# Blaizzy/mlx-audio-swift

Measured on AMD Instinct MI355X. Metric: audio-seconds/sec (TTS gen+codec decode), Orpheus-3B batch 32 per GPU: value = whole-job aggregate over n_gpus, value_per_gpu = value / n_gpus, higher is better.
Workload: dtype bf16

## Files before the change

### include/mi_speech_debug.h

```cpp
#ifndef MI_SPEECH_DEBUG_H
#define MI_SPEECH_DEBUG_H
#include "mi_speech.h"
#ifdef __cplusplus
extern "C" {
#endif

mis_status mis_debug_launch_floor(int device, int n_kernels, int mode, int reps, double* us_per_kernel);
int32_t mis_debug_choose_split(int32_t items, int32_t k_tiles, int32_t waves_per_item, int32_t s_max);
mis_status mis_debug_occupy_cus(int device, int blocks, int threads, double seconds);
mis_status mis_debug_occupy_wait(void);
int32_t mis_debug_device_cus(int device);
int32_t mis_debug_sampler_failures(void);
int64_t mis_debug_whisper_weight_bytes(const mis_whisper* c);
mis_status mis_debug_mimi_decoder_tap(mis_mimi* m, const int32_t* codes, int batch, int n_q, int T, int stage, float* out, int64_t capacity,
                                      int32_t* channels, int64_t* length);

mis_status mis_debug_gemm_skinny(int device, const uint16_t* W, const uint16_t* W2, const uint16_t* X, const uint16_t* bias, int M, int N, int K,
                                 int epi, int R, int ksb, int U, int S, float* out, int64_t capacity, int32_t* report);
mis_status mis_debug_gemm_skinny_q(int device, int bits, int sb_dtype, const uint32_t* wq, const uint16_t* scales, const uint16_t* biases,
                                   const uint32_t* wq2, const uint16_t* scales2, const uint16_t* biases2, const uint16_t* X, const uint16_t* bias,
                                   int M, int N, int K, int epi, int R, int ksb, int S, float* out, int64_t capacity, int32_t* report);
mis_status mis_debug_gemm_pf(int device, const uint16_t* W, const uint16_t* W2, const uint16_t* X, const uint16_t* h, int M, int N, int K, int epi,
                             float* out, int64_t capacity, int32_t* report);

typedef struct mis_debug_attn_args {
    int32_t batch, Mpad, S, Nqkv, H, Hkv, D, Smax;
    int32_t cache_rows, append_only, first_schedule, cross, cross_len, out_ld, rope_in_dtype;
    int32_t qp_S, qp_KT;
    float scale, qk_eps, qp_eps;
    const float* qkv_part;
    const int32_t* pos;
    const uint8_t* active;
    const float *rope_cos, *rope_sin;
    const uint16_t *qnorm_w, *knorm_w;
    const uint16_t* qp_w;
    const uint16_t* qp_bias;
    const float* qp_slabs;
    const uint16_t *qp_h_in, *qp_lnw, *qp_lnb;
    const uint16_t *kcache, *vtcache;
    uint16_t *kcache_out, *vtcache_out;
    float* out;
    uint16_t* qp_h_out;
    int32_t* report;
} mis_debug_attn_args;
mis_status mis_debug_attn_decode(int device, const mis_debug_attn_args* args);

mis_status mis_debug_token_engine(mis_tts* lm, const int32_t* prompt, int n_prompt, int n_new, int xcds, const mis_gen_params* sampling,
                                  int stop_id, int32_t* next_tokens, float* logits_out, float* hidden_out, int32_t* counts, double* ms_out);

mis_status mis_debug_marvis_forced_logits(mis_marvis* c, const int32_t* tokens, const uint8_t* mask, const int32_t* prompt_lens, int P,
                                          int batch, const mis_marvis_params* params, const int32_t* forced, int F, float* logits_out,
                                          int32_t* sampled_out, int32_t* n_frames);
mis_status mis_debug_marvis_sample_logits(int device, const float* logits, int batch, int vocab, float temperature, float top_p,
                                          uint64_t seed, int64_t row_offset, int frame, int slot, int K, int32_t* tokens_out);
mis_status mis_debug_marvis_rope_tables(int head_dim, float theta, float factor, float low_freq_factor, float high_freq_factor,
                                        float old_context_len, int n_pos, float* cos_out, float* sin_out);

mis_status mis_debug_moonshine_stem_tap(mis_moonshine* c, const float* pcm, const int64_t* lens, int batch, int64_t stride, int stage,
                                        float* out, int64_t capacity, int64_t* dims);

mis_status mis_debug_smartturn_tap(mis_smartturn* c, int stage, float* out, int64_t capacity);
mis_status mis_debug_smartturn_timing(const mis_smartturn* c, float* ms);

mis_status mis_debug_ecapa_lid_timing(const mis_ecapa_lid* c, float* ms);

#ifdef __cplusplus
}
#endif
#endif
```

### mlx-audio-swift_amd/_lib.py

```python
from __future__ import annotations

import ctypes as C
import os

_HERE = os.path.dirname(os.path.abspath(__file__))
LIB_PATH = os.environ.get("MIS_LIB_PATH") or os.path.join(_HERE, "libmi_speech.so")

MIS_OK = 0
STATUS_NAMES = {0: "ok", 1: "modelNotInitialized", 2: "generationFailed", 3: "invalidInput",
                4: "audioDecodingFailed", 5: "audioEncodingFailed", 6: "cancelled", 7: "device"}
MIS_F32, MIS_F16, MIS_BF16, MIS_I32 = 0, 1, 2, 3
EVENT_TOKEN, EVENT_INFO, EVENT_AUDIO = 0, 1, 2


class SnacConfigC(C.Structure):
    _fields_ = [("sampling_rate", C.c_int32), ("latent_dim", C.c_int32), ("decoder_dim", C.c_int32),
                ("n_decoder_rates", C.c_int32), ("decoder_rates", C.c_int32 * 8), ("codebook_size", C.c_int32),
                ("codebook_dim", C.c_int32), ("n_codebooks", C.c_int32), ("vq_strides", C.c_int32 * 8),
                ("noise", C.c_int32), ("depthwise", C.c_int32), ("attn_window_size", C.c_int32)]


class LmConfigC(C.Structure):
    _fields_ = [("hidden_size", C.c_int32), ("num_hidden_layers", C.c_int32), ("intermediate_size", C.c_int32),
                ("num_attention_heads", C.c_int32), ("num_key_value_heads", C.c_int32), ("head_dim", C.c_int32),
# ... 321 lines not shown
    "mis_encodec_hop_length": (C.c_int, [_P]),
    "mis_encodec_decode_frame": (C.c_int, [_P, _P, C.c_int, C.c_int, C.c_int, _P, _P]),
    "mis_encodec_debug_tap": (C.c_int, [_P, _P, C.c_int, C.c_int, C.c_int, C.c_int, _P, C.c_int64, C.POINTER(C.c_int32),
                                        C.POINTER(C.c_int64)]),
    "mis_mimi_202407": (None, [C.c_int, C.POINTER(MimiConfigC)]),
    "mis_mimi_create": (C.c_int, [C.POINTER(MimiConfigC), C.c_int, C.POINTER(_P)]),
    "mis_mimi_set_tensor": (C.c_int, [_P, C.c_char_p, _P, C.c_int, C.POINTER(C.c_int64), C.c_int]),
    "mis_mimi_finalize": (C.c_int, [_P]),
    "mis_mimi_destroy": (None, [_P]),
    "mis_mimi_num_samples": (C.c_int64, [_P, C.c_int]),
    "mis_mimi_decode": (C.c_int, [_P, _P, C.c_int, C.c_int, C.c_int, _P]),
    "mis_mimi_encode_num_frames": (C.c_int64, [_P, C.c_int64]),
    "mis_mimi_encode": (C.c_int, [_P, _P, C.c_int, C.c_int64, C.c_int, _P]),
    "mis_mimi_decode_stream_begin": (C.c_int, [_P, C.c_int]),
    "mis_mimi_decode_stream_step": (C.c_int, [_P, _P, C.c_int, C.c_int, _P]),
    "mis_mimi_decode_stream_end": (C.c_int, [_P]),
    "mis_marvis_create": (C.c_int, [C.POINTER(MarvisConfigC), C.c_int, C.POINTER(_P)]),
    "mis_marvis_set_tensor": (C.c_int, [_P, C.c_char_p, _P, C.c_int, C.POINTER(C.c_int64), C.c_int]),
    "mis_marvis_set_tensor_quantized": (C.c_int, [_P, C.c_char_p, _P, _P, _P, C.c_int, C.c_int64, C.c_int64, C.c_int, C.c_int]),
    "mis_marvis_init_synthetic": (C.c_int, [_P, C.c_uint64]),
    "mis_marvis_init_synthetic_quantized": (C.c_int, [_P, C.c_uint64, C.c_int]),
    "mis_marvis_finalize": (C.c_int, [_P]),
    "mis_marvis_destroy": (None, [_P]),
    "mis_marvis_backbone": (_P, [_P]),
    "mis_marvis_decoder": (_P, [_P]),
    "mis_marvis_launches_per_frame": (C.c_int, [_P]),
    "mis_marvis_generate_codes": (C.c_int, [_P, _P, _P, _P, C.c_int, C.c_int, C.POINTER(MarvisParamsC), _P, C.POINTER(_P),
                                            C.POINTER(C.c_int64), _P]),
    "mis_marvis_generate": (C.c_int, [_P, _P, _P, _P, _P, C.c_int, C.c_int, C.POINTER(MarvisParamsC), _P, C.POINTER(_P),
                                      C.POINTER(C.c_int64), _P, C.POINTER(_P), C.POINTER(C.c_int64), _P, C.c_int, _P, _P, _P]),
}

class AttnDebugArgsC(C.Structure):
    _fields_ = ([(n, C.c_int32) for n in ("batch", "Mpad", "S", "Nqkv", "H", "Hkv", "D", "Smax", "cache_rows", "append_only", "first_schedule",
                                          "cross", "cross_len", "out_ld", "rope_in_dtype", "qp_S", "qp_KT")] +
                [(n, C.c_float) for n in ("scale", "qk_eps", "qp_eps")] +
                [(n, _P) for n in ("qkv_part", "pos", "active", "rope_cos", "rope_sin", "qnorm_w", "knorm_w", "qp_w", "qp_bias", "qp_slabs",
                                   "qp_h_in", "qp_lnw", "qp_lnb", "kcache", "vtcache", "kcache_out", "vtcache_out", "out", "qp_h_out", "report")])


DEBUG_SYMBOLS = {
    "mis_debug_launch_floor": (C.c_int, [C.c_int, C.c_int, C.c_int, C.c_int, C.POINTER(C.c_double)]),
    "mis_debug_occupy_cus": (C.c_int, [C.c_int, C.c_int, C.c_int, C.c_double]),
    "mis_debug_occupy_wait": (C.c_int, []),
    "mis_debug_device_cus": (C.c_int32, [C.c_int]),
    "mis_debug_sampler_failures": (C.c_int32, []),
    "mis_debug_choose_split": (C.c_int32, [C.c_int32, C.c_int32, C.c_int32, C.c_int32]),
    "mis_debug_gemm_skinny": (C.c_int, [C.c_int, _P, _P, _P, _P, C.c_int, C.c_int, C.c_int, C.c_int, C.c_int, C.c_int, C.c_int, C.c_int, _P,
                                        C.c_int64, _P]),
    "mis_debug_gemm_skinny_q": (C.c_int, [C.c_int, C.c_int, C.c_int, _P, _P, _P, _P, _P, _P, _P, _P, C.c_int, C.c_int, C.c_int, C.c_int, C.c_int,
                                          C.c_int, C.c_int, _P, C.c_int64, _P]),
    "mis_debug_gemm_pf": (C.c_int, [C.c_int, _P, _P, _P, _P, C.c_int, C.c_int, C.c_int, C.c_int, _P, C.c_int64, _P]),
    "mis_debug_attn_decode": (C.c_int, [C.c_int, C.POINTER(AttnDebugArgsC)]),
    "mis_debug_token_engine": (C.c_int, [_P, _P, C.c_int, C.c_int, C.c_int, _P, C.c_int, _P, _P, _P, _P, C.POINTER(C.c_double)]),
    "mis_debug_whisper_weight_bytes": (C.c_int64, [_P]),
    "mis_debug_mimi_decoder_tap": (C.c_int, [_P, _P, C.c_int, C.c_int, C.c_int, C.c_int, _P, C.c_int64, C.POINTER(C.c_int32),
                                             C.POINTER(C.c_int64)]),
    "mis_debug_marvis_forced_logits": (C.c_int, [_P, _P, _P, _P, C.c_int, C.c_int, C.POINTER(MarvisParamsC), _P, C.c_int, _P, _P, _P]),
    "mis_debug_marvis_sample_logits": (C.c_int, [C.c_int, _P, C.c_int, C.c_int, C.c_float, C.c_float, C.c_uint64, C.c_int64, C.c_int,
                                                 C.c_int, C.c_int, _P]),
    "mis_debug_moonshine_stem_tap": (C.c_int, [_P, _P, _P, C.c_int, C.c_int64, C.c_int, _P, C.c_int64, _P]),
    "mis_debug_smartturn_tap": (C.c_int, [_P, C.c_int, _P, C.c_int64]),
    "mis_debug_smartturn_timing": (C.c_int, [_P, _P]),
    "mis_debug_ecapa_lid_timing": (C.c_int, [_P, _P]),
    "mis_debug_marvis_rope_tables": (C.c_int, [C.c_int, C.c_float, C.c_float, C.c_float, C.c_float, C.c_float, C.c_int, _P, _P]),
}

_lib = None


class MisLibraryMissing(RuntimeError):
    pass


def lib():
    global _lib
    if _lib is None:
        if not os.path.exists(LIB_PATH):
            raise MisLibraryMissing(
                f"{LIB_PATH} not found: build it with `python -c 'import __graft_entry__ as g; g.build()'` "
                "(hipcc --offload-arch=gfx950). There is no CPU fallback.")
        try:
            import torch
        except Exception:
            pass
        l = C.CDLL(LIB_PATH)
        for name, (res, args) in list(SYMBOLS.items()) + list(DEBUG_SYMBOLS.items()):
            fn = getattr(l, name)
            fn.restype = res
            fn.argtypes = args
        _lib = l
    return _lib


def last_error() -> str:
    m = lib().mis_last_error()
    return m.decode("utf-8", "replace") if m else ""
```

### mlx-audio-swift_amd/csrc/lm_kernels.hip

```cpp
#include <hip/hip_fp16.h>
#include "common.h"
#include <algorithm>
#include <type_traits>
#include <string>
#include "lm_kernels.h"



__global__ void k_convert_to_bf16(const void* __restrict__ src, int dtype, bf16_t* __restrict__ dst, size_t n) {
    size_t i = (size_t)blockIdx.x * blockDim.x + threadIdx.x;
    if (i >= n) return;
    if (dtype == MIS_F32) dst[i] = f32_to_bf16(((const float*)src)[i]);
    else if (dtype == MIS_F16) dst[i] = f32_to_bf16((float)((const _Float16*)src)[i]);
    else dst[i] = ((const bf16_t*)src)[i];
}

__global__ void k_bf16_to_f32(const bf16_t* __restrict__ src, float* __restrict__ dst, size_t n) {
    size_t i = (size_t)blockIdx.x * blockDim.x + threadIdx.x;
    if (i < n) dst[i] = bf16_to_f32(src[i]);
}

__global__ void k_pack_weight(const bf16_t* __restrict__ src, bf16_t* __restrict__ dst, int N, int K, int NT,
                              int tile_stride, int tile_offset) {
    int KT = K / 32;
// ... 225 lines not shown
        for (int k = 0; k < RR_MAXC; ++k) {
            int i = c0 + tid + k * RR_THREADS;
            keep[k] = 0.0f;
            if (i < N) {
                float o = bf16_round_f32(acc[k]);
                float hn = bf16_round_f32(hv[k] + o);
                h[(size_t)m * N + i] = f32_to_bf16(hn);
                keep[k] = hn;
                ss += hn * hn;
            }
        }
    }
    if (ln_bias) {
        float sum = 0.0f;
        if (N <= RR_THREADS * RR_MAXC) {
#pragma unroll
            for (int k = 0; k < RR_MAXC; ++k) sum += keep[k];
        } else {
            for (int i = tid; i < N; i += RR_THREADS) sum += bf16_to_f32(h[(size_t)m * N + i]);
        }
        const float mean = block_sum_1024(sum, red) / (float)N;
        float sq = 0.0f;
        if (N <= RR_THREADS * RR_MAXC) {
#pragma unroll
            for (int k = 0; k < RR_MAXC; ++k) {
                int i = tid + k * RR_THREADS;
                if (i < N) { float dlt = keep[k] - mean; sq += dlt * dlt; }
            }
        } else {
            for (int i = tid; i < N; i += RR_THREADS) { float dlt = bf16_to_f32(h[(size_t)m * N + i]) - mean; sq += dlt * dlt; }
        }
        const float rstd = 1.0f / sqrtf(block_sum_1024(sq, red) / (float)N + eps);
        for (int i = tid; i < N; i += RR_THREADS) {
            float f = bf16_to_f32(h[(size_t)m * N + i]);
            x[xpk_index(m, i, MT)] = f32_to_bf16((f - mean) * rstd * bf16_to_f32(wnorm[i]) + bf16_to_f32(ln_bias[i]));
        }
        return;
    }
    float tot = block_sum_1024(ss, red);
    float inv = 1.0f / sqrtf(tot / (float)N + eps);
    if (N <= RR_THREADS * RR_MAXC) {
#pragma unroll
        for (int k = 0; k < RR_MAXC; ++k) {
            int i = tid + k * RR_THREADS;
            if (i < N) x[xpk_index(m, i, MT)] = f32_to_bf16(wv[k] * bf16_round_f32(keep[k] * inv));
        }
    } else {
        for (int i = tid; i < N; i += RR_THREADS) {
            float f = bf16_to_f32(h[(size_t)m * N + i]);
            x[xpk_index(m, i, MT)] = f32_to_bf16(bf16_to_f32(wnorm[i]) * bf16_round_f32(f * inv));
        }
    }
}
template <int SG, bool LN>
__global__ void __launch_bounds__(1024) k_glue4(const float* __restrict__ slabs, int S, int Mpad, int N, bf16_t* __restrict__ h,
                                                const bf16_t* __restrict__ wnorm, bf16_t* __restrict__ x, float eps,
                                                const bf16_t* __restrict__ ln_bias) {
    __shared__ float red[16];
    const int m = blockIdx.x, tid = threadIdx.x, nth = blockDim.x;
    const int MT = Mpad >> 4;
    const int c4 = tid < (N >> 2) ? tid : (N >> 2) - 1;
    const bool live = tid < (N >> 2);
    unsigned long long hq, wq, bq = 0;
    f32x4_t v[SG];
    {
        const bf16_t* hp = h + (size_t)m * N + 4 * c4;
        const bf16_t* wp = wnorm + 4 * c4;
        asm volatile("global_load_dwordx2 %0, %1, off" : "=v"(hq) : "v"(hp));
        asm volatile("global_load_dwordx2 %0, %1, off" : "=v"(wq) : "v"(wp));
        if constexpr (LN) {
            const bf16_t* bp = ln_bias + 4 * c4;
            asm volatile("global_load_dwordx2 %0, %1, off" : "=v"(bq) : "v"(bp));
        }
#pragma unroll
        for (int j = 0; j < SG; ++j) {
            const int sj = j < S ? j : S - 1;
            const float* sp = slabs + ((size_t)sj * Mpad + m) * N + 4 * c4;
            asm volatile("global_load_dwordx4 %0, %1, off" : "=v"(v[j]) : "v"(sp));
        }
        if constexpr (SG == 2) asm volatile("s_waitcnt vmcnt(0)" : "+v"(hq), "+v"(wq), "+v"(v[0]), "+v"(v[1]));
        else if constexpr (SG == 4) asm volatile("s_waitcnt vmcnt(0)" : "+v"(hq), "+v"(wq), "+v"(v[0]), "+v"(v[1]), "+v"(v[2]), "+v"(v[3]));
        else asm volatile("s_waitcnt vmcnt(0)" : "+v"(hq), "+v"(wq), "+v"(v[0]), "+v"(v[1]), "+v"(v[2]), "+v"(v[3]), "+v"(v[4]), "+v"(v[5]),
                          "+v"(v[6]), "+v"(v[7]));
        if constexpr (LN) asm volatile("" : "+v"(bq));
    }
    float acc[4] = {0.f, 0.f, 0.f, 0.f};
#pragma unroll
    for (int j = 0; j < SG; ++j) {
        const bool on = j < S;
        acc[0] += on ? v[j][0] : 0.0f; acc[1] += on ? v[j][1] : 0.0f; acc[2] += on ? v[j][2] : 0.0f; acc[3] += on ? v[j][3] : 0.0f;
    }
    const uint32_t hq0 = (uint32_t)hq, hq1 = (uint32_t)(hq >> 32);
    const float hv[4] = {bf16_to_f32((bf16_t)(hq0 & 0xffffu)), bf16_to_f32((bf16_t)(hq0 >> 16)), bf16_to_f32((bf16_t)(hq1 & 0xffffu)),
                         bf16_to_f32((bf16_t)(hq1 >> 16))};
    const uint32_t wq0 = (uint32_t)wq, wq1 = (uint32_t)(wq >> 32);
    const float wv[4] = {bf16_to_f32((bf16_t)(wq0 & 0xffffu)), bf16_to_f32((bf16_t)(wq0 >> 16)), bf16_to_f32((bf16_t)(wq1 & 0xffffu)),
                         bf16_to_f32((bf16_t)(wq1 >> 16))};
    float hn[4], ss = 0.0f;
    bf16_t hb[4];
#pragma unroll
    for (int e = 0; e < 4; ++e) {
        hn[e] = bf16_round_f32(hv[e] + bf16_round_f32(acc[e]));
        hb[e] = f32_to_bf16(hn[e]);
        ss += live ? hn[e] * hn[e] : 0.0f;
    }
    if (live) *reinterpret_cast<uint2*>(h + (size_t)m * N + 4 * c4) =
        make_uint2((uint32_t)hb[0] | ((uint32_t)hb[1] << 16), (uint32_t)hb[2] | ((uint32_t)hb[3] << 16));
    if constexpr (LN) {
        float sm = 0.0f;
#pragma unroll
        for (int e = 0; e < 4; ++e) sm += live ? hn[e] : 0.0f;
        sm = wave_sum_dpp(sm);
        if ((tid & 63) == 0) red[tid >> 6] = sm;
        __syncthreads();
        float tot = 0.0f;
        const int nw = nth >> 6;
#pragma unroll
        for (int i = 0; i < 16; ++i) tot += i < nw ? red[i] : 0.0f;
        const float mean = tot / (float)N;
        float sq = 0.0f;
#pragma unroll
        for (int e = 0; e < 4; ++e) { const float dl = hn[e] - mean; sq += live ? dl * dl : 0.0f; }
        sq = wave_sum_dpp(sq);
        __syncthreads();
        if ((tid & 63) == 0) red[tid >> 6] = sq;
        __syncthreads();
        float tq = 0.0f;
#pragma unroll
        for (int i = 0; i < 16; ++i) tq += i < nw ? red[i] : 0.0f;
        const float rstd = 1.0f / sqrtf(tq / (float)N + eps);
        if (live) {
            const uint32_t bq0 = (uint32_t)bq, bq1 = (uint32_t)(bq >> 32);
            const float bv[4] = {bf16_to_f32((bf16_t)(bq0 & 0xffffu)), bf16_to_f32((bf16_t)(bq0 >> 16)), bf16_to_f32((bf16_t)(bq1 & 0xffffu)),
                                 bf16_to_f32((bf16_t)(bq1 >> 16))};
            bf16_t xb[4];
#pragma unroll
            for (int e = 0; e < 4; ++e) xb[e] = f32_to_bf16((hn[e] - mean) * rstd * wv[e] + bv[e]);
            *reinterpret_cast<uint2*>(x + xpk_index(m, 4 * c4, MT)) =
                make_uint2((uint32_t)xb[0] | ((uint32_t)xb[1] << 16), (uint32_t)xb[2] | ((uint32_t)xb[3] << 16));
        }
        return;
    }
    ss = wave_sum_dpp(ss);
    if ((tid & 63) == 0) red[tid >> 6] = ss;
    __syncthreads();
    float tot = 0.0f;
    const int nw = nth >> 6;
#pragma unroll
    for (int i = 0; i < 16; ++i) tot += i < nw ? red[i] : 0.0f;
    const float inv = 1.0f / sqrtf(tot / (float)N + eps);
    if (live) {
        bf16_t xb[4];
#pragma unroll
        for (int e = 0; e < 4; ++e) xb[e] = f32_to_bf16(wv[e] * bf16_round_f32(hn[e] * inv));
        *reinterpret_cast<uint2*>(x + xpk_index(m, 4 * c4, MT)) =
            make_uint2((uint32_t)xb[0] | ((uint32_t)xb[1] << 16), (uint32_t)xb[2] | ((uint32_t)xb[3] << 16));
    }
}

template <int SG, int CPT, bool LN>
__global__ void __launch_bounds__(256) k_glue_cpt(const float* __restrict__ slabs, int S, int Mpad, int N, bf16_t* __restrict__ h,
                                                  const bf16_t* __restrict__ wnorm, bf16_t* __restrict__ x, float eps, const bf16_t* __restrict__ ln_bias) {
    __shared__ float red[4];
    const int m = blockIdx.x, tid = threadIdx.x, nth = blockDim.x;
    const int MT = Mpad >> 4;
    const int nw = nth >> 6;
    unsigned long long hq[CPT], wq[CPT], bq[CPT];
    f32x4_t v[CPT][SG];
#pragma unroll
    for (int g = 0; g < CPT; ++g) {
        const int c4 = tid + g * nth;
        const bf16_t* hp = h + (size_t)m * N + 4 * c4;
        const bf16_t* wp = wnorm + 4 * c4;
        asm volatile("global_load_dwordx2 %0, %1, off" : "=v"(hq[g]) : "v"(hp));
        asm volatile("global_load_dwordx2 %0, %1, off" : "=v"(wq[g]) : "v"(wp));
        if constexpr (LN) {
            const bf16_t* bp = ln_bias + 4 * c4;
            asm volatile("global_load_dwordx2 %0, %1, off" : "=v"(bq[g]) : "v"(bp));
        } else bq[g] = 0;
    }
#pragma unroll
    for (int j = 0; j < SG; ++j) {
        const int sj = j < S ? j : S - 1;
#pragma unroll
        for (int g = 0; g < CPT; ++g) {
            const float* sp = slabs + ((size_t)sj * Mpad + m) * N + 4 * (tid + g * nth);
            asm volatile("global_load_dwordx4 %0, %1, off" : "=v"(v[g][j]) : "v"(sp));
        }
    }
    asm volatile("s_waitcnt vmcnt(0)" ::: "memory");
#pragma unroll
    for (int g = 0; g < CPT; ++g) {
        asm volatile("" : "+v"(hq[g]), "+v"(wq[g]));
        if constexpr (LN) asm volatile("" : "+v"(bq[g]));
#pragma unroll
        for (int j = 0; j < SG; ++j) asm volatile("" : "+v"(v[g][j]));
    }
    auto row_sum = [&](float part, bool again) {
        part = wave_sum_dpp(part);
        if (nw == 1) return part;
        if (again) __syncthreads();
        if ((tid & 63) == 0) red[tid >> 6] = part;
        __syncthreads();
        float tot = 0.0f;
#pragma unroll
        for (int i = 0; i < 4; ++i) tot += i < nw ? red[i] : 0.0f;
        return tot;
    };
    float hn[CPT][4], wv[CPT][4], ss = 0.0f, sm = 0.0f;
#pragma unroll
    for (int g = 0; g < CPT; ++g) {
        float acc[4] = {0.f, 0.f, 0.f, 0.f};
#pragma unroll
        for (int j = 0; j < SG; ++j) {
            const bool on = j < S;
            acc[0] += on ? v[g][j][0] : 0.0f; acc[1] += on ? v[g][j][1] : 0.0f; acc[2] += on ? v[g][j][2] : 0.0f; acc[3] += on ? v[g][j][3] : 0.0f;
        }
        const uint32_t h0 = (uint32_t)hq[g], h1 = (uint32_t)(hq[g] >> 32), w0 = (uint32_t)wq[g], w1 = (uint32_t)(wq[g] >> 32);
        const float hv[4] = {bf16_to_f32((bf16_t)(h0 & 0xffffu)), bf16_to_f32((bf16_t)(h0 >> 16)), bf16_to_f32((bf16_t)(h1 & 0xffffu)), bf16_to_f32((bf16_t)(h1 >> 16))};
        wv[g][0] = bf16_to_f32((bf16_t)(w0 & 0xffffu)); wv[g][1] = bf16_to_f32((bf16_t)(w0 >> 16));
        wv[g][2] = bf16_to_f32((bf16_t)(w1 & 0xffffu)); wv[g][3] = bf16_to_f32((bf16_t)(w1 >> 16));
        bf16_t hb[4];
#pragma unroll
        for (int e = 0; e < 4; ++e) {
            hn[g][e] = bf16_round_f32(hv[e] + bf16_round_f32(acc[e]));
            hb[e] = f32_to_bf16(hn[g][e]);
            ss += hn[g][e] * hn[g][e];
            sm += hn[g][e];
        }
        *reinterpret_cast<uint2*>(h + (size_t)m * N + 4 * (tid + g * nth)) =
            make_uint2((uint32_t)hb[0] | ((uint32_t)hb[1] << 16), (uint32_t)hb[2] | ((uint32_t)hb[3] << 16));
    }
    if constexpr (LN) {
        const float mean = row_sum(sm, false) / (float)N;
        float sq = 0.0f;
#pragma unroll
        for (int g = 0; g < CPT; ++g)
#pragma unroll
            for (int e = 0; e < 4; ++e) { const float dl = hn[g][e] - mean; sq += dl * dl; }
        const float rstd = 1.0f / sqrtf(row_sum(sq, true) / (float)N + eps);
#pragma unroll
// ... 942 lines not shown
        if (xs_nj == 6) xs_run(std::integral_constant<int, 6>{});
        else xs_run(std::integral_constant<int, 5>{});
#undef XS_BIND
    } else {
        for (int tile = wave; tile < n_tiles; tile += 2 * ATT_WAVES) {
            const int tile2 = tile + ATT_WAVES;
            const bool has2 = tile2 < n_tiles;
            if (tile != wave) {
                load_tile(tile, kA, vA);
                if (has2) load_tile(tile2, kB, vB);
            }
            if (tile == new_tile) patch_new_key(kA, vA);
            process(tile, kA, vA);
            if (has2) {
                if (tile2 == new_tile) patch_new_key(kB, vB);
                process(tile2, kB, vB);
            }
        }
    }
    ATT_STAMP(5);
    l_run += __shfl_xor(l_run, 16, 64);
    l_run += __shfl_xor(l_run, 32, 64);
    if (g4 == 0) { sm[wave * 16 + h] = m_run; sl[wave * 16 + h] = l_run; }
#pragma unroll
    for (int r = 0; r < 4; ++r) {
        int head = g4 * 4 + r;
        if (head < G) {
#pragma unroll
            for (int dt = 0; dt < D / 16; ++dt) sO[((size_t)wave * G + head) * D + dt * 16 + h] = O[dt][r];
        }
    }
    __syncthreads();
    ATT_STAMP(6);
    for (int idx = tid; idx < G * D; idx += 512) {
        int head = idx / D, d = idx - head * D;
        float M = -INFINITY;
#pragma unroll
        for (int w = 0; w < ATT_WAVES; ++w) M = fmaxf(M, sm[w * 16 + head]);
        float num = 0.0f, den = 0.0f;
#pragma unroll
        for (int w = 0; w < ATT_WAVES; ++w) {
            float f = __expf(sm[w * 16 + head] - M);
            num += f * sO[((size_t)w * G + head) * D + d];
            den += f * sl[w * 16 + head];
        }
        const bf16_t ov = f32_to_bf16(num / den);
        if (p.out_ld) p.out[(size_t)b * p.out_ld + (kvh * G + head) * D + d] = ov;
        else p.out[xpk_index(b, (kvh * G + head) * D + d, p.Mpad >> 4)] = ov;
    }
    ATT_STAMP(7);
}

#define ATT2_MAX_J 4
__device__ __forceinline__ void att2_issue_tile(const bf16_t* kt, const bf16_t* vt, unsigned voff, bf16x8_t (&ka)[2][4], bf16x8_t (&vb)[8]) {
    const bf16_t* kt1 = kt + 4 * 512;
    const bf16_t* vt1 = vt + 4 * 512;
#define ATT2_NT " nt"
#define ATT2_LD(DST, BASE, OFF) asm volatile("global_load_dwordx4 %0, %1, %2 offset:" #OFF ATT2_NT : "=v"(DST) : "v"(voff), "s"(BASE))
    asm volatile("s_nop 4\n\tglobal_load_dwordx4 %0, %1, %2" ATT2_NT : "=v"(ka[0][0]) : "v"(voff), "s"(kt));
    ATT2_LD(ka[0][1], kt, 1024); ATT2_LD(ka[0][2], kt, 2048); ATT2_LD(ka[0][3], kt, 3072);
    asm volatile("s_nop 4\n\tglobal_load_dwordx4 %0, %1, %2" ATT2_NT : "=v"(ka[1][0]) : "v"(voff), "s"(kt1));
    ATT2_LD(ka[1][1], kt1, 1024); ATT2_LD(ka[1][2], kt1, 2048); ATT2_LD(ka[1][3], kt1, 3072);
    asm volatile("s_nop 4\n\tglobal_load_dwordx4 %0, %1, %2" ATT2_NT : "=v"(vb[0]) : "v"(voff), "s"(vt));
    ATT2_LD(vb[1], vt, 1024); ATT2_LD(vb[2], vt, 2048); ATT2_LD(vb[3], vt, 3072);
    asm volatile("s_nop 4\n\tglobal_load_dwordx4 %0, %1, %2" ATT2_NT : "=v"(vb[4]) : "v"(voff), "s"(vt1));
    ATT2_LD(vb[5], vt1, 1024); ATT2_LD(vb[6], vt1, 2048); ATT2_LD(vb[7], vt1, 3072);
#undef ATT2_LD
}
#define ATT2_VMCNT(CNT) asm volatile("s_waitcnt vmcnt(" #CNT ")" ::: "memory")
#define ATT2_BIND_TILE(KA, VB)                                                                                               \
    asm volatile("" : "+v"(KA[0][0]), "+v"(KA[0][1]), "+v"(KA[0][2]), "+v"(KA[0][3]), "+v"(KA[1][0]), "+v"(KA[1][1]), "+v"(KA[1][2]),  \
                      "+v"(KA[1][3]), "+v"(VB[0]), "+v"(VB[1]), "+v"(VB[2]), "+v"(VB[3]), "+v"(VB[4]), "+v"(VB[5]), "+v"(VB[6]), "+v"(VB[7]))

template <int NS>
__global__ void __launch_bounds__(512) k_attn_decode2(AttnParams p) {
    constexpr int D = 128;
    extern __shared__ __attribute__((aligned(16))) unsigned char smem[];
    const int kvh = blockIdx.x, b = blockIdx.y;
    const int tid = threadIdx.x, lane = tid & 63, wave = __builtin_amdgcn_readfirstlane(tid >> 6);
    const int G = p.H / p.Hkv;
    float* strip = reinterpret_cast<float*>(smem) + (size_t)wave * 7 * D;
    float* sm = reinterpret_cast<float*>(smem) + (size_t)ATT_WAVES * 7 * D;
    float* sl = sm + ATT_WAVES * 16;
    float* sO = sl + ATT_WAVES * 16;

    const uint32_t active_word = reinterpret_cast<const uint32_t*>(p.active)[b >> 2];
    const unsigned char row_active = (unsigned char)((active_word >> (8 * (b & 3))) & 0xffu);
    const int pos = p.pos[b];
    if (!row_active) return;
    const int kv_len = pos + 1;
    const int n_tiles = (kv_len + 31) >> 5;
    const int new_tile = pos >> 5;
    const bool owner = (new_tile & (ATT_WAVES - 1)) == wave;
    const int nj = wave < n_tiles ? (n_tiles - wave + ATT_WAVES - 1) / ATT_WAVES : 0;

    bf16_t* kc = p.kcache + ((size_t)(b * p.Hkv + kvh) * p.Smax) * D;
    bf16_t* vt = p.vtcache + ((size_t)(b * p.Hkv + kvh) * D) * p.Smax;
    const unsigned voff = (unsigned)lane * 16u;
    auto ktile = [&](int tile) { return kc + (size_t)tile * 32 * D; };
    auto vtile = [&](int tile) { return vt + (size_t)tile * 32 * D; };
    const int h = lane & 15, g4 = lane >> 4;
    const int pr = pos & 31;
    const int prow = ((pr >> 3) << 2) | (pr & 3), phalf = (pr >> 2) & 1;
    bf16_t* kro = reinterpret_cast<bf16_t*>(strip + 6 * D);

    f32x4_t O[D / 16];
// ... 86 lines not shown
        __builtin_amdgcn_wave_barrier();
        __builtin_amdgcn_fence(__ATOMIC_ACQUIRE, "wavefront");

#pragma unroll
        for (int dt = 0; dt < D / 16; ++dt) O[dt] = (f32x4_t){0.f, 0.f, 0.f, 0.f};
        m_run = -INFINITY; l_run = 0.0f;
        auto process = [&](int tile, const bf16x8_t (&ka)[2][4], const bf16x8_t (&vb)[8]) {
            const int base = tile * 32;
            f32x4_t S0 = (f32x4_t){0.f, 0.f, 0.f, 0.f}, S1 = S0;
#pragma unroll
            for (int c = 0; c < D / 32; ++c) {
                S0 = __builtin_amdgcn_mfma_f32_16x16x32_bf16(ka[0][c], qf[c], S0, 0, 0, 0);
                S1 = __builtin_amdgcn_mfma_f32_16x16x32_bf16(ka[1][c], qf[c], S1, 0, 0, 0);
            }
            float sc[8];
            float mx = -INFINITY;
#pragma unroll
            for (int e = 0; e < 8; ++e) {
                float v = (e < 4 ? S0[e] : S1[e - 4]) * p.scale;
                v = (base + g4 * 8 + e < kv_len) ? v : -INFINITY;
                sc[e] = v;
                mx = fmaxf(mx, v);
            }
            mx = fmaxf(mx, __shfl_xor(mx, 16, 64));
            mx = fmaxf(mx, __shfl_xor(mx, 32, 64));
            float m_new = fmaxf(m_run, mx);
            float alpha = __expf(m_run - m_new);
            float psum = 0.0f;
            bf16x8_t ph, pl;
#pragma unroll
            for (int e = 0; e < 8; ++e) {
                float pe = __expf(sc[e] - m_new);
                psum += pe;
                bf16_t hi = f32_to_bf16(pe);
                bf16_t lo = f32_to_bf16(pe - bf16_to_f32(hi));
                ph[e] = (short)hi;
                pl[e] = (short)lo;
            }
            l_run = l_run * alpha + psum;
            m_run = m_new;
            float ar[4];
#pragma unroll
            for (int r = 0; r < 4; ++r) ar[r] = __shfl(alpha, g4 * 4 + r, 64);
#pragma unroll
            for (int dt = 0; dt < D / 16; ++dt) {
                f32x4_t o = O[dt];
#pragma unroll
                for (int r = 0; r < 4; ++r) o[r] *= ar[r];
                o = __builtin_amdgcn_mfma_f32_16x16x32_bf16(ph, vb[dt], o, 0, 0, 0);
                o = __builtin_amdgcn_mfma_f32_16x16x32_bf16(pl, vb[dt], o, 0, 0, 0);
                O[dt] = o;
            }
        };
        auto last = [&](int tile, bf16x8_t (&ka)[2][4], bf16x8_t (&vb)[8]) {
            if (owner) {
                if ((lane & 15) == prow) {
                    bf16x8_t* dst = reinterpret_cast<bf16x8_t*>(kc) + ((size_t)new_tile * 2 + phalf) * (D / 32) * 64 + lane;
#pragma unroll
                    for (int c = 0; c < 4; ++c) {
                        const bf16x8_t kn = *reinterpret_cast<const bf16x8_t*>(kro + c * 32 + g4 * 8);
                        if (phalf) ka[1][c] = kn; else ka[0][c] = kn;
                        dst[c * 64] = kn;
                    }
                }
                if ((lane >> 4) == (pr >> 3)) {
#pragma unroll
                    for (int dt = 0; dt < 8; ++dt) {
                        const bf16_t vn = f32_to_bf16(strip[(G + 1) * D + dt * 16 + (lane & 15)]);
#pragma unroll
                        for (int e = 0; e < 8; ++e)
                            if (e == (pr & 7)) vb[dt][e] = (short)vn;
                        vt[(((size_t)new_tile * (D / 16) + dt) * 64 + lane) * 8 + (pr & 7)] = vn;
                    }
                }
            }
            process(tile, ka, vb);
        };
        __builtin_amdgcn_sched_barrier(0);
        if constexpr (NJ >= 2) att2_issue_tile(ktile(wave + ATT_WAVES), vtile(wave + ATT_WAVES), voff, kB, vB);
        if constexpr (NJ >= 1) {
            if constexpr (NJ >= 2) ATT2_VMCNT(16); else ATT2_VMCNT(0);
            ATT2_BIND_TILE(kA, vA);
            __builtin_amdgcn_sched_barrier(0);
            if constexpr (NJ == 1) last(wave, kA, vA); else process(wave, kA, vA);
            __builtin_amdgcn_sched_barrier(0);
        }
        if constexpr (NJ >= 2) {
            if constexpr (NJ >= 3) att2_issue_tile(ktile(wave + 2 * ATT_WAVES), vtile(wave + 2 * ATT_WAVES), voff, kA, vA);
            if constexpr (NJ >= 3) ATT2_VMCNT(16); else ATT2_VMCNT(0);
            ATT2_BIND_TILE(kB, vB);
            __builtin_amdgcn_sched_barrier(0);
            if constexpr (NJ == 2) last(wave + ATT_WAVES, kB, vB); else process(wave + ATT_WAVES, kB, vB);
            __builtin_amdgcn_sched_barrier(0);
        }
        if constexpr (NJ >= 3) {
            if constexpr (NJ >= 4) att2_issue_tile(ktile(wave + 3 * ATT_WAVES), vtile(wave + 3 * ATT_WAVES), voff, kB, vB);
            if constexpr (NJ >= 4) ATT2_VMCNT(16); else ATT2_VMCNT(0);
            ATT2_BIND_TILE(kA, vA);
            __builtin_amdgcn_sched_barrier(0);
            if constexpr (NJ == 3) last(wave + 2 * ATT_WAVES, kA, vA); else process(wave + 2 * ATT_WAVES, kA, vA);
            __builtin_amdgcn_sched_barrier(0);
        }
        if constexpr (NJ >= 4) {
            ATT2_VMCNT(0);
            ATT2_BIND_TILE(kB, vB);
            __builtin_amdgcn_sched_barrier(0);
            last(wave + 3 * ATT_WAVES, kB, vB);
        }
    };
    switch (nj) {
        case 1: run(std::integral_constant<int, 1>{}); break;
        case 2: run(std::integral_constant<int, 2>{}); break;
        case 3: run(std::integral_constant<int, 3>{}); break;
        case 4: run(std::integral_constant<int, 4>{}); break;
        default: run(std::integral_constant<int, 0>{}); break;
    }
    l_run += __shfl_xor(l_run, 16, 64);
    l_run += __shfl_xor(l_run, 32, 64);
    if (g4 == 0) { sm[wave * 16 + h] = m_run; sl[wave * 16 + h] = l_run; }
#pragma unroll
    for (int r = 0; r < 4; ++r) {
        int head = g4 * 4 + r;
        if (head < G) {
#pragma unroll
            for (int dt = 0; dt < D / 16; ++dt) sO[((size_t)wave * G + head) * D + dt * 16 + h] = O[dt][r];
        }
    }
    __syncthreads();
    for (int idx = tid; idx < G * D; idx += 512) {
        int head = idx / D, d = idx - head * D;
        float M = -INFINITY;
#pragma unroll
        for (int w = 0; w < ATT_WAVES; ++w) M = fmaxf(M, sm[w * 16 + head]);
        float num = 0.0f, den = 0.0f;
#pragma unroll
        for (int w = 0; w < ATT_WAVES; ++w) {
            float f = __expf(sm[w * 16 + head] - M);
            num += f * sO[((size_t)w * G + head) * D + d];
            den += f * sl[w * 16 + head];
        }
        const bf16_t ov = f32_to_bf16(num / den);
        if (p.out_ld) p.out[(size_t)b * p.out_ld + (kvh * G + head) * D + d] = ov;
        else p.out[xpk_index(b, (kvh * G + head) * D + d, p.Mpad >> 4)] = ov;
    }
}
static size_t attn2_smem_bytes(int G) { return ((size_t)ATT_WAVES * 7 * 128 + 2 * ATT_WAVES * 16 + (size_t)ATT_WAVES * G * 128) * 4; }

#ifdef MIS_ATTN_TIMING
#include <string.h>
static unsigned long long* g_attn_dbg = nullptr;
static int g_attn_slot = 0;
extern "C" int mis_debug_attn_timing_init() {
    if (!g_attn_dbg) {
        if (hipHostMalloc((void**)&g_attn_dbg, 4096 * 16 * sizeof(unsigned long long), 0) != hipSuccess) return 1;
        memset(g_attn_dbg, 0, 4096 * 16 * 8);
    }
    g_attn_slot = 0;
    return 0;
}
extern "C" int mis_debug_attn_timing(unsigned long long* out, int max_slots) {
    int n = g_attn_slot < max_slots ? g_attn_slot : max_slots;
    if (g_attn_dbg) memcpy(out, g_attn_dbg, (size_t)n * 16 * 8);
    return n;
}
#endif
static int attn_nit(int G, int D) {
    const int n_el = (G + 2) * D;
    return n_el <= 1024 ? 2 : (D == 128 ? 5 : 3);
}
size_t attn_smem_bytes(int G, int D) {
    return (size_t)attn_nit(G, D) * 512 * 4 + 16 * D * 2 + D * 2 + 2 * ATT_WAVES * 16 * 4 + (size_t)ATT_WAVES * G * D * 4;
}

thread_local AttnLaunchInfo g_attn_last_launch;

bool attn_qp_ok(const AttnParams& p) {
    const char* xe = getenv("MIS_ATTN_XS");
    return !(xe && atoi(xe) == 0) && p.cross && p.D == 64 && p.H == p.Hkv && !p.append_only && !p.cache_rows && !p.rope_cos && !p.qnorm_w &&
           (p.cross_len + 31) / 32 >= ATT_WAVES * ATT_XS_MIN_J && (p.cross_len + 31) / 32 <= ATT_WAVES * ATT_XS_MAX_J && p.qp_KT >= 1 &&
           (p.qp_KT + ATT_WAVES - 1) / ATT_WAVES <= ATT_QP_KW && p.qp_KT * 32 == p.H * p.D && p.qp_S >= 1 && p.qp_S <= 8;
}
void launch_attn_decode(const AttnParams& p, int batch, hipStream_t s) {
    int G = p.H / p.Hkv;
    MIS_REQUIRE(G >= 1 && G <= 16 && p.H % p.Hkv == 0, MIS_ERR_INVALID_INPUT, "GQA group size must be 1..16");
    size_t smem = attn_smem_bytes(G, p.D);
    MIS_REQUIRE(smem <= 64 * 1024, MIS_ERR_INVALID_INPUT, "attention LDS footprint too large");
    MIS_REQUIRE(p.qp_w || (p.S >= 1 && p.S <= 8), MIS_ERR_GENERATION_FAILED, "attention prologue reduces at most 8 split-K slabs (got %d)", p.S);
    MIS_REQUIRE(((uintptr_t)p.active & 3) == 0, MIS_ERR_GENERATION_FAILED, "attention: the active-flag array must be 4-byte aligned");
    MIS_REQUIRE(!p.qp_w || attn_qp_ok(p), MIS_ERR_GENERATION_FAILED, "attention: the query-projection prologue does not apply to this launch");
    MIS_REQUIRE(p.Smax >= 32 && p.Smax % 32 == 0, MIS_ERR_INVALID_INPUT, "attention: %d cache positions are not a multiple of the 32-key tile", p.Smax);
    dim3 grid(p.Hkv, batch), block(512);
    const int n_el = (G + 2) * p.D;
    if (!p.first_schedule && !p.cache_rows && !p.append_only && p.D == 128 && !p.cross && p.rope_cos && !p.rope_in_dtype && !p.qnorm_w && p.S <= 4 && G <= 4 && p.Smax <= 32 * ATT_WAVES * ATT2_MAX_J &&
        p.Smax % 32 == 0 && ((uintptr_t)p.qkv_part & 15) == 0 && p.Nqkv % 4 == 0) {
        const size_t sm2 = attn2_smem_bytes(G);
        MIS_REQUIRE((p.Smax / 32 + ATT_WAVES - 1) / ATT_WAVES <= ATT2_MAX_J, MIS_ERR_GENERATION_FAILED,
// ... 43 lines not shown
```

Baseline: 184.1.

## Vectorize attention combine, precompute new KV tile data, use SGPR-base glue loads

The glue residual-RMSNorm kernels now issue loads with a scalar base and a 32-bit vector offset instead of full 64-bit per-lane addresses, which cuts VGPR address arithmetic. The decode attention kernel gathers the new token's K/V values early (prep) and merges them into the last tile with branch-free masked selects, so that work overlaps the outstanding tile loads. The cross-wave combine is also vectorized: each thread handles 8 output columns with 16-byte LDS reads and stores, and the sm/sl layout is transposed to head-major to allow this. A debug entry point for the glue kernel is added. The risks are extra register pressure and the more complex masking logic.

```diff
diff --git a/include/mi_speech_debug.h b/include/mi_speech_debug.h
--- a/include/mi_speech_debug.h
+++ b/include/mi_speech_debug.h
@@ -45,6 +45,9 @@
 } mis_debug_attn_args;
 mis_status mis_debug_attn_decode(int device, const mis_debug_attn_args* args);
 
+mis_status mis_debug_glue(int device, const float* slabs, int S, int Mpad, int N, const uint16_t* h_in, const uint16_t* wnorm,
+                          const uint16_t* ln_bias, float eps, uint16_t* h_out, uint16_t* x_out);
+
 mis_status mis_debug_token_engine(mis_tts* lm, const int32_t* prompt, int n_prompt, int n_new, int xcds, const mis_gen_params* sampling,
                                   int stop_id, int32_t* next_tokens, float* logits_out, float* hidden_out, int32_t* counts, double* ms_out);
 
diff --git a/mlx-audio-swift_amd/_lib.py b/mlx-audio-swift_amd/_lib.py
--- a/mlx-audio-swift_amd/_lib.py
+++ b/mlx-audio-swift_amd/_lib.py
@@ -397,6 +397,7 @@
                                           C.c_int, C.c_int, _P, C.c_int64, _P]),
     "mis_debug_gemm_pf": (C.c_int, [C.c_int, _P, _P, _P, _P, C.c_int, C.c_int, C.c_int, C.c_int, _P, C.c_int64, _P]),
     "mis_debug_attn_decode": (C.c_int, [C.c_int, C.POINTER(AttnDebugArgsC)]),
+    "mis_debug_glue": (C.c_int, [C.c_int, _P, C.c_int, C.c_int, C.c_int, _P, _P, _P, C.c_float, _P, _P]),
     "mis_debug_token_engine": (C.c_int, [_P, _P, C.c_int, C.c_int, C.c_int, _P, C.c_int, _P, _P, _P, _P, C.POINTER(C.c_double)]),
     "mis_debug_whisper_weight_bytes": (C.c_int64, [_P]),
     "mis_debug_mimi_decoder_tap": (C.c_int, [_P, _P, C.c_int, C.c_int, C.c_int, C.c_int, _P, C.c_int64, C.POINTER(C.c_int32),
diff --git a/mlx-audio-swift_amd/csrc/glue_debug.hip b/mlx-audio-swift_amd/csrc/glue_debug.hip
--- /dev/null
+++ b/mlx-audio-swift_amd/csrc/glue_debug.hip
@@ -0,0 +1,34 @@
+#include "common.h"
+#include "lm_kernels.h"
+#include "debug_guard.h"
+#include "../../include/mi_speech_debug.h"
+
+extern "C" mis_status mis_debug_glue(int device, const float* slabs, int S, int Mpad, int N, const uint16_t* h_in, const uint16_t* wnorm,
+                                     const uint16_t* ln_bias, float eps, uint16_t* h_out, uint16_t* x_out) {
+    MIS_API_BEGIN
+    MIS_REQUIRE(slabs && h_in && wnorm && h_out && x_out, MIS_ERR_INVALID_INPUT, "glue: slabs, h, the norm weight and both outputs are required");
+    MIS_REQUIRE(S >= 1 && S <= 64 && Mpad >= 16 && Mpad % 16 == 0 && Mpad <= 64 && N >= 32 && N % 32 == 0 && N <= 16384, MIS_ERR_INVALID_INPUT,
+                "glue: 1 <= S <= 64 slabs, Mpad 16 .. 64 (a multiple of 16), N a multiple of 32 up to 16384");
+    HIP_CHECK(hipSetDevice(device));
+    DevBuf<uint32_t> d_slabs;
+    DevBuf<uint16_t> d_w, d_b;
+    alloc32(d_slabs, slabs, (size_t)S * Mpad * N, F32_NAN);
+    alloc16(d_w, wnorm, N, BF16_NAN);
+    if (ln_bias) alloc16(d_b, ln_bias, N, BF16_NAN);
+    GuardedOut h, x;
+    const size_t bytes = (size_t)Mpad * N * 2;
+    h.alloc(bytes, (size_t)N * 2);
+    x.alloc(bytes, (size_t)N * 2);
+    HIP_CHECK(hipMemcpy(h.p(), h_in, bytes, hipMemcpyHostToDevice));
+    launch_reduce_residual_rmsnorm(reinterpret_cast<const float*>(d_slabs.p), S, Mpad, N, reinterpret_cast<bf16_t*>(h.p()), d_w.p,
+                                   reinterpret_cast<bf16_t*>(x.p()), eps, 0, ln_bias ? d_b.p : nullptr);
+    HIP_CHECK(hipGetLastError());
+    HIP_CHECK(hipDeviceSynchronize());
+    h.check_guards(); x.check_guards();
+    HIP_CHECK(hipMemcpy(h_out, h.p(), bytes, hipMemcpyDeviceToHost));
+    std::vector<uint16_t> pk((size_t)Mpad * N);
+    HIP_CHECK(hipMemcpy(pk.data(), x.p(), bytes, hipMemcpyDeviceToHost));
+    for (int m = 0; m < Mpad; ++m)
+        for (int k = 0; k < N; ++k) x_out[(size_t)m * N + k] = pk[xpk_index(m, k, Mpad >> 4)];
+    MIS_API_END
+}
diff --git a/mlx-audio-swift_amd/csrc/lm_kernels.hip b/mlx-audio-swift_amd/csrc/lm_kernels.hip
--- a/mlx-audio-swift_amd/csrc/lm_kernels.hip
+++ b/mlx-audio-swift_amd/csrc/lm_kernels.hip
@@ -301,6 +301,8 @@
         }
     }
 }
+#define GLUE_LD(OP, DST, VOFF, BASE) asm volatile(OP " %0, %1, %2" : "=v"(DST) : "v"(VOFF), "s"(BASE))
+#define GLUE_LD_S(OP, DST, VOFF, BASE) asm volatile("s_nop 4\n\t" OP " %0, %1, %2" : "=v"(DST) : "v"(VOFF), "s"(BASE))
 template <int SG, bool LN>
 __global__ void __launch_bounds__(1024) k_glue4(const float* __restrict__ slabs, int S, int Mpad, int N, bf16_t* __restrict__ h,
                                                 const bf16_t* __restrict__ wnorm, bf16_t* __restrict__ x, float eps,
@@ -313,19 +315,17 @@
     unsigned long long hq, wq, bq = 0;
     f32x4_t v[SG];
     {
-        const bf16_t* hp = h + (size_t)m * N + 4 * c4;
-        const bf16_t* wp = wnorm + 4 * c4;
-        asm volatile("global_load_dwordx2 %0, %1, off" : "=v"(hq) : "v"(hp));
-        asm volatile("global_load_dwordx2 %0, %1, off" : "=v"(wq) : "v"(wp));
-        if constexpr (LN) {
-            const bf16_t* bp = ln_bias + 4 * c4;
-            asm volatile("global_load_dwordx2 %0, %1, off" : "=v"(bq) : "v"(bp));
-        }
+        const unsigned o8 = 8u * (unsigned)c4, o16 = 16u * (unsigned)c4;
+        const bf16_t* hrow = h + (size_t)m * N;
+        const float* srow = slabs + (size_t)m * N;
+        const size_t slab_stride = (size_t)Mpad * N;
+        GLUE_LD_S("global_load_dwordx2", hq, o8, hrow);
+        GLUE_LD("global_load_dwordx2", wq, o8, wnorm);
+        if constexpr (LN) GLUE_LD("global_load_dwordx2", bq, o8, ln_bias);
 #pragma unroll
         for (int j = 0; j < SG; ++j) {
-            const int sj = j < S ? j : S - 1;
-            const float* sp = slabs + ((size_t)sj * Mpad + m) * N + 4 * c4;
-            asm volatile("global_load_dwordx4 %0, %1, off" : "=v"(v[j]) : "v"(sp));
+            const float* sp = srow + (size_t)(j < S ? j : S - 1) * slab_stride;
+            GLUE_LD("global_load_dwordx4", v[j], o16, sp);
         }
         if constexpr (SG == 2) asm volatile("s_waitcnt vmcnt(0)" : "+v"(hq), "+v"(wq), "+v"(v[0]), "+v"(v[1]));
         else if constexpr (SG == 4) asm volatile("s_waitcnt vmcnt(0)" : "+v"(hq), "+v"(wq), "+v"(v[0]), "+v"(v[1]), "+v"(v[2]), "+v"(v[3]));
@@ -416,26 +416,25 @@
     const int nw = nth >> 6;
     unsigned long long hq[CPT], wq[CPT], bq[CPT];
     f32x4_t v[CPT][SG];
+    unsigned o8[CPT], o16[CPT];
+#pragma unroll
+    for (int g = 0; g < CPT; ++g) { o8[g] = 8u * (unsigned)(tid + g * nth); o16[g] = 2u * o8[g]; }
+    const bf16_t* hrow = h + (size_t)m * N;
+    const float* srow = slabs + (size_t)m * N;
+    const size_t slab_stride = (size_t)Mpad * N;
 #pragma unroll
     for (int g = 0; g < CPT; ++g) {
-        const int c4 = tid + g * nth;
-        const bf16_t* hp = h + (size_t)m * N + 4 * c4;
-        const bf16_t* wp = wnorm + 4 * c4;
-        asm volatile("global_load_dwordx2 %0, %1, off" : "=v"(hq[g]) : "v"(hp));
-        asm volatile("global_load_dwordx2 %0, %1, off" : "=v"(wq[g]) : "v"(wp));
-        if constexpr (LN) {
-            const bf16_t* bp = ln_bias + 4 * c4;
-            asm volatile("global_load_dwordx2 %0, %1, off" : "=v"(bq[g]) : "v"(bp));
-        } else bq[g] = 0;
+        if (g == 0) GLUE_LD_S("global_load_dwordx2", hq[g], o8[g], hrow);
+        else GLUE_LD("global_load_dwordx2", hq[g], o8[g], hrow);
+        GLUE_LD("global_load_dwordx2", wq[g], o8[g], wnorm);
+        if constexpr (LN) GLUE_LD("global_load_dwordx2", bq[g], o8[g], ln_bias);
+        else bq[g] = 0;
     }
 #pragma unroll
     for (int j = 0; j < SG; ++j) {
-        const int sj = j < S ? j : S - 1;
-#pragma unroll
-        for (int g = 0; g < CPT; ++g) {
-            const float* sp = slabs + ((size_t)sj * Mpad + m) * N + 4 * (tid + g * nth);
-            asm volatile("global_load_dwordx4 %0, %1, off" : "=v"(v[g][j]) : "v"(sp));
-        }
+        const float* sp = srow + (size_t)(j < S ? j : S - 1) * slab_stride;
+#pragma unroll
+        for (int g = 0; g < CPT; ++g) GLUE_LD("global_load_dwordx4", v[g][j], o16[g], sp);
     }
     asm volatile("s_waitcnt vmcnt(0)" ::: "memory");
 #pragma unroll
@@ -1484,6 +1483,8 @@
 }
 
 #define ATT2_MAX_J 4
+#define ATT2_CW 8
+typedef uint32_t u32x4_t __attribute__((ext_vector_type(4)));
 __device__ __forceinline__ void att2_issue_tile(const bf16_t* kt, const bf16_t* vt, unsigned voff, bf16x8_t (&ka)[2][4], bf16x8_t (&vb)[8]) {
     const bf16_t* kt1 = kt + 4 * 512;
     const bf16_t* vt1 = vt + 4 * 512;
@@ -1676,26 +1677,47 @@
                 O[dt] = o;
             }
         };
+        bf16x8_t knew[4];
+        uint32_t vnew[8], vmask[4], ksel;
+        auto prep = [&]() {
+#pragma unroll
+            for (int c = 0; c < 4; ++c) knew[c] = *reinterpret_cast<const bf16x8_t*>(kro + c * 32 + g4 * 8);
+#pragma unroll
+            for (int dt = 0; dt < 8; ++dt) {
+                const uint32_t vn = f32_to_bf16(strip[(G + 1) * D + dt * 16 + (lane & 15)]);
+                vnew[dt] = vn | (vn << 16);
+            }
+            const uint32_t half = g4 == (pr >> 3) ? ((pr & 1) ? 0xffff0000u : 0x0000ffffu) : 0u;
+#pragma unroll
+            for (int j = 0; j < 4; ++j) vmask[j] = j == ((pr & 7) >> 1) ? half : 0u;
+            asm volatile("" : "+v"(knew[0]), "+v"(knew[1]), "+v"(knew[2]), "+v"(knew[3]));
+            asm volatile("" : "+v"(vnew[0]), "+v"(vnew[1]), "+v"(vnew[2]), "+v"(vnew[3]), "+v"(vnew[4]), "+v"(vnew[5]), "+v"(vnew[6]), "+v"(vnew[7]));
+            ksel = (lane & 15) == prow ? 1u + (uint32_t)phalf : 0u;
+            asm volatile("" : "+v"(vmask[0]), "+v"(vmask[1]), "+v"(vmask[2]), "+v"(vmask[3]), "+v"(ksel));
+        };
         auto last = [&](int tile, bf16x8_t (&ka)[2][4], bf16x8_t (&vb)[8]) {
             if (owner) {
-                if ((lane & 15) == prow) {
+#pragma unroll
+                for (int c = 0; c < 4; ++c) {
+                    ka[0][c] = ksel == 1u ? knew[c] : ka[0][c];
+                    ka[1][c] = ksel == 2u ? knew[c] : ka[1][c];
+                }
+#pragma unroll
+                for (int dt = 0; dt < 8; ++dt) {
+                    u32x4_t w = (u32x4_t)vb[dt];
+#pragma unroll
+                    for (int j = 0; j < 4; ++j) w[j] = (vmask[j] & vnew[dt]) | (~vmask[j] & w[j]);
+                    vb[dt] = (bf16x8_t)w;
+                }
+                if (ksel) {
                     bf16x8_t* dst = reinterpret_cast<bf16x8_t*>(kc) + ((size_t)new_tile * 2 + phalf) * (D / 32) * 64 + lane;
 #pragma unroll
-                    for (int c = 0; c < 4; ++c) {
-                        const bf16x8_t kn = *reinterpret_cast<const bf16x8_t*>(kro + c * 32 + g4 * 8);
-                        if (phalf) ka[1][c] = kn; else ka[0][c] = kn;
-                        dst[c * 64] = kn;
-                    }
+                    for (int c = 0; c < 4; ++c) dst[c * 64] = knew[c];
                 }
                 if ((lane >> 4) == (pr >> 3)) {
 #pragma unroll
-                    for (int dt = 0; dt < 8; ++dt) {
-                        const bf16_t vn = f32_to_bf16(strip[(G + 1) * D + dt * 16 + (lane & 15)]);
-#pragma unroll
-                        for (int e = 0; e < 8; ++e)
-                            if (e == (pr & 7)) vb[dt][e] = (short)vn;
-                        vt[(((size_t)new_tile * (D / 16) + dt) * 64 + lane) * 8 + (pr & 7)] = vn;
-                    }
+                    for (int dt = 0; dt < 8; ++dt)
+                        vt[(((size_t)new_tile * (D / 16) + dt) * 64 + lane) * 8 + (pr & 7)] = (bf16_t)(vnew[dt] & 0xffffu);
                 }
             }
             process(tile, ka, vb);
@@ -1703,6 +1725,7 @@
         __builtin_amdgcn_sched_barrier(0);
         if constexpr (NJ >= 2) att2_issue_tile(ktile(wave + ATT_WAVES), vtile(wave + ATT_WAVES), voff, kB, vB);
         if constexpr (NJ >= 1) {
+            if constexpr (NJ == 1) prep();
             if constexpr (NJ >= 2) ATT2_VMCNT(16); else ATT2_VMCNT(0);
             ATT2_BIND_TILE(kA, vA);
             __builtin_amdgcn_sched_barrier(0);
@@ -1711,6 +1734,7 @@
         }
         if constexpr (NJ >= 2) {
             if constexpr (NJ >= 3) att2_issue_tile(ktile(wave + 2 * ATT_WAVES), vtile(wave + 2 * ATT_WAVES), voff, kA, vA);
+            if constexpr (NJ == 2) prep();
             if constexpr (NJ >= 3) ATT2_VMCNT(16); else ATT2_VMCNT(0);
             ATT2_BIND_TILE(kB, vB);
             __builtin_amdgcn_sched_barrier(0);
@@ -1719,6 +1743,7 @@
         }
         if constexpr (NJ >= 3) {
             if constexpr (NJ >= 4) att2_issue_tile(ktile(wave + 3 * ATT_WAVES), vtile(wave + 3 * ATT_WAVES), voff, kB, vB);
+            if constexpr (NJ == 3) prep();
             if constexpr (NJ >= 4) ATT2_VMCNT(16); else ATT2_VMCNT(0);
             ATT2_BIND_TILE(kA, vA);
             __builtin_amdgcn_sched_barrier(0);
@@ -1726,6 +1751,7 @@
             __builtin_amdgcn_sched_barrier(0);
         }
         if constexpr (NJ >= 4) {
+            prep();
             ATT2_VMCNT(0);
             ATT2_BIND_TILE(kB, vB);
             __builtin_amdgcn_sched_barrier(0);
@@ -1741,7 +1767,7 @@
     }
     l_run += __shfl_xor(l_run, 16, 64);
     l_run += __shfl_xor(l_run, 32, 64);
-    if (g4 == 0) { sm[wave * 16 + h] = m_run; sl[wave * 16 + h] = l_run; }
+    if (g4 == 0) { sm[h * ATT_WAVES + wave] = m_run; sl[h * ATT_WAVES + wave] = l_run; }
 #pragma unroll
     for (int r = 0; r < 4; ++r) {
         int head = g4 * 4 + r;
@@ -1751,21 +1777,49 @@
         }
     }
     __syncthreads();
-    for (int idx = tid; idx < G * D; idx += 512) {
-        int head = idx / D, d = idx - head * D;
+    constexpr int CW = ATT2_CW;
+    static_assert(ATT_WAVES == 8 && (CW == 8 || CW == 4), "combine: two 16-byte reads of sm / sl per head, 16- or 8-byte output stores");
+    if (tid < G * (D / CW)) {
+        const int head = tid / (D / CW), d0 = (tid - head * (D / CW)) * CW;
+        float mw[ATT_WAVES], lw[ATT_WAVES];
+#pragma unroll
+        for (int q = 0; q < 2; ++q) {
+            const f32x4_t mq = *reinterpret_cast<const f32x4_t*>(sm + head * ATT_WAVES + 4 * q);
+            const f32x4_t lq = *reinterpret_cast<const f32x4_t*>(sl + head * ATT_WAVES + 4 * q);
+#pragma unroll
+            for (int e = 0; e < 4; ++e) { mw[4 * q + e] = mq[e]; lw[4 * q + e] = lq[e]; }
+        }
         float M = -INFINITY;
 #pragma unroll
-        for (int w = 0; w < ATT_WAVES; ++w) M = fmaxf(M, sm[w * 16 + head]);
-        float num = 0.0f, den = 0.0f;
+        for (int w = 0; w < ATT_WAVES; ++w) M = fmaxf(M, mw[w]);
+        float num[CW], den = 0.0f;
+#pragma unroll
+        for (int e = 0; e < CW; ++e) num[e] = 0.0f;
 #pragma unroll
         for (int w = 0; w < ATT_WAVES; ++w) {
-            float f = __expf(sm[w * 16 + head] - M);
-            num += f * sO[((size_t)w * G + head) * D + d];
-            den += f * sl[w * 16 + head];
-        }
-        const bf16_t ov = f32_to_bf16(num / den);
-        if (p.out_ld) p.out[(size_t)b * p.out_ld + (kvh * G + head) * D + d] = ov;
-        else p.out[xpk_index(b, (kvh * G + head) * D + d, p.Mpad >> 4)] = ov;
+            const float f = __expf(mw[w] - M);
+            const float* so = sO + ((size_t)w * G + head) * D + d0;
+#pragma unroll
+            for (int q = 0; q < CW / 4; ++q) {
+                const f32x4_t x = *reinterpret_cast<const f32x4_t*>(so + 4 * q);
+#pragma unroll
+                for (int e = 0; e < 4; ++e) num[4 * q + e] += f * x[e];
+            }
+            den += f * lw[w];
+        }
+        uint32_t ow[CW / 2];
+#pragma unroll
+        for (int e = 0; e < CW / 2; ++e)
+            ow[e] = (uint32_t)f32_to_bf16(num[2 * e] / den) | ((uint32_t)f32_to_bf16(num[2 * e + 1] / den) << 16);
+        const int col = (kvh * G + head) * D + d0;
+        bf16_t* op = p.out_ld ? p.out + (size_t)b * p.out_ld + col : p.out + xpk_index(b, col, p.Mpad >> 4);
+        if (!p.out_ld || (p.out_ld & (CW - 1)) == 0) {
+            if constexpr (CW == 8) *reinterpret_cast<u32x4_t*>(op) = (u32x4_t){ow[0], ow[1], ow[CW / 2 - 2], ow[CW / 2 - 1]};
+            else *reinterpret_cast<uint2*>(op) = make_uint2(ow[0], ow[1]);
+        } else {
+#pragma unroll
+            for (int e = 0; e < CW; ++e) op[e] = (bf16_t)(ow[e >> 1] >> (16 * (e & 1)));
+        }
     }
 }
 static size_t attn2_smem_bytes(int G) { return ((size_t)ATT_WAVES * 7 * 128 + 2 * ATT_WAVES * 16 + (size_t)ATT_WAVES * G * 128) * 4; }
```

Result: no change. 183.9 (-0.1%).
